# jchristopherson/nonlin

Hardware: AMD Instinct MI355X
Metric: LM iterations/sec on m=4096,n=256 fp64; FD-Jacobian GB/s vs HBM peak (higher is better)
Workload: dtype f64

## Files before the change

include/nonlin_hip.h:

```cpp
#ifndef NONLIN_HIP_H
#define NONLIN_HIP_H

#include <stdint.h>

#ifdef __cplusplus
extern "C" {
#endif

#define NLH_NO_ERROR                     0
#define NLH_INVALID_INPUT_ERROR        201
#define NLH_ARRAY_SIZE_ERROR           202
#define NLH_OUT_OF_MEMORY_ERROR        105
#define NLH_INVALID_OPERATION_ERROR    104
#define NLH_CONVERGENCE_ERROR          106
#define NLH_DIVERGENT_BEHAVIOR_ERROR   206
#define NLH_SPURIOUS_CONVERGENCE_ERROR 207
#define NLH_TOLERANCE_TOO_SMALL_ERROR  208
#define NLH_DIVIDE_BY_ZERO_ERROR       210
#define NLH_UNDEFINED_FUNCTION_ERROR   211
#define NLH_UNDERDEFINED_PROBLEM_ERROR 212
#define NLH_ERR_NO_DEVICE             -1
#define NLH_ERR_HIP                   -2
#define NLH_ERR_BAD_HANDLE            -3

// ... 205 lines not shown
                    double *dA, double *db, double *dxtrue, double *dx0);


int nlh_dq_residual(nlh_handle *h, int32_t nprob, int32_t m, int32_t n, const double *dA,
                    const double *db, double gamma, const double *dx, double *df);
int nlh_dq_fd_panel(nlh_handle *h, int32_t nprob, int32_t m, int32_t n, const double *dA,
                    const double *db, double gamma, const double *dx, double *dP);
int nlh_fd_jacobian_panel(nlh_handle *h, int32_t nprob, int32_t m, int32_t n,
                          const double *dP, const double *df0, const double *dx, double *dJ);
int nlh_dq_jacobian(nlh_handle *h, int32_t nprob, int32_t m, int32_t n, const double *dA,
                    double gamma, const double *dx, double *dJ);
int nlh_gram(nlh_handle *h, int32_t nprob, int32_t m, int32_t n, const double *dJ,
             const double *df, double *dG, double *dg);
int nlh_chol_factor(nlh_handle *h, int32_t nprob, int32_t n, double *dG, const double *dg,
                    int32_t *dipvt, double *dacnorm, double *dqtf, int32_t *dinfo);
int nlh_qr_factor(nlh_handle *h, int32_t nprob, int32_t m, int32_t n, double *dJ,
                  const double *df, int32_t *dipvt, double *drdiag, double *dacnorm,
                  double *dqtf, double *dwa4);
int nlh_lmfactor_exact(nlh_handle *h, int32_t nprob, int32_t m, int32_t n, const double *dJ,
                       const double *df, double *dR, int32_t *dipvt, double *drdiag, double *dacnorm,
                       double *dqtf, double *dwa4);
enum { NLH_QRX_SWEEP_COLUMN = 0,
       NLH_QRX_SWEEP_LANE = 1 };
enum { NLH_QRX_INIT_SPLIT = 0,
       NLH_QRX_INIT_FUSED = 1 };
enum { NLH_QRX_PIVOT_FEW32 = 0,
       NLH_QRX_PIVOT_BATCH32 = 1,
       NLH_QRX_PIVOT_FEW64 = 2,
       NLH_QRX_PIVOT_BATCH64 = 3,
       NLH_QRX_PIVOT_LONG = 4,
       NLH_QRX_PIVOT_LONG_SCALED = 5,
       NLH_QRX_PIVOT_LONG_SPLIT = 6 };
enum { NLH_QRX_PASS_COLUMN = 0,
       NLH_QRX_PASS_WIDE = 1,
       NLH_QRX_PASS_WIDE_HALF = 2,
       NLH_QRX_PASS_FOUR_WAVE = 3,
       NLH_QRX_PASS_WAVE = 4,
       NLH_QRX_PASS_WAVE_SHARED = 5 };
typedef struct nlh_qrx_plan_head {
    int32_t sweep, init;
    int32_t use_list, ny;
    int32_t nact;
} nlh_qrx_plan_head;
typedef struct nlh_qrx_plan_step {
    int32_t j, cur, np;
    int32_t lo;
    int32_t flush, pf;
    int32_t pivot, pass;
    int32_t gwin;
    int32_t lds, lds_max;
} nlh_qrx_plan_step;
int32_t nlh_qrx_plan(int32_t nprob, int32_t m, int32_t n, int32_t nact, int32_t have_stages,
                     nlh_qrx_plan_head *head, nlh_qrx_plan_step *steps, int32_t cap);
int nlh_lmpar(nlh_handle *h, int32_t nprob, int32_t n, double *dR, int32_t ldr,
              const int32_t *dipvt, const double *ddiag, const double *dqtf,
              const double *ddelta, const double *dtailsq, double *dpar,
              double *dxstep, double *dsdiag);
int nlh_lu_factor(nlh_handle *h, int32_t nprob, int32_t n, double *dA, int32_t *dipvt,
                  int32_t *dinfo);
int nlh_lu_solve(nlh_handle *h, int32_t nprob, int32_t n, const double *dLU,
                 const int32_t *dipvt, double *db);
int nlh_qr_factor_full(nlh_handle *h, int32_t nprob, int32_t n, const double *dB, double *dQ,
                       double *dRt);
int nlh_qr_rank1_update(nlh_handle *h, int32_t nprob, int32_t n, double *dQ, double *dRt,
                        const double *du, const double *dv);
int nlh_solve_upper(nlh_handle *h, int32_t nprob, int32_t n, const double *dRt, double *dx);
int nlh_chol_rank1(nlh_handle *h, int32_t n, int32_t downdate, double *dRt, double *du, int32_t *hinfo);

int nlh_poly_fit(nlh_handle *h, int32_t npts, int32_t order, int32_t thru_zero, const double *x,
                 const double *y, double *coef);
int nlh_poly_fit_batch(nlh_handle *h, int32_t nprob, int32_t npts, int32_t order, int32_t thru_zero,
                       const double *dx, const double *dy, double *dcoef);

int nlh_poly_roots(nlh_handle *h, int32_t order, const double *coef, double *z, int32_t *info);
int nlh_poly_roots_batch(nlh_handle *h, int32_t nprob, int32_t order, const double *dcoef, double *dz,
                         int32_t *dinfo);
int nlh_poly_eval_batch(nlh_handle *h, int32_t nprob, int32_t order, int32_t npts, const double *dcoef,
                        const double *dx, double *dy);
int nlh_poly_eval_complex_batch(nlh_handle *h, int32_t nprob, int32_t order, int32_t npts, const double *dcoef,
                                const double *dz, double *dy);

int nlh_covar(nlh_handle *h, int32_t nprob, int32_t n, const double *dR, const int32_t *dipvt, double tol,
              double *dcov, int32_t *drank);
int64_t nlh_covar_lds_bytes(int32_t n);
int nlh_lm_covariance_batch_device(nlh_handle *h, int32_t nprob, int32_t m, int32_t n, nlh_device_vecfcn fcn,
                                   nlh_device_jacfcn jacfcn, void *ctx, const double *dx, int32_t scaled, double tol,
                                   double *dcov, double *dsigma, int32_t *drank, double *dchi2);
int nlh_lm_covariance_batch_device_h(nlh_handle *h, int32_t nprob, int32_t m, int32_t n, nlh_device_vecfcn fcn,
                                     nlh_device_jacfcn jacfcn, void *ctx, const double *x, int32_t scaled, double tol,
                                     double *cov, double *sigma, int32_t *rank, double *chi2);
int nlh_lm_covariance(nlh_handle *h, int32_t m, int32_t n, nlh_vecfcn fcn, nlh_jacfcn jacfcn, void *ctx, double *x,
                      int32_t scaled, double tol, double *cov, double *sigma, int32_t *rank, double *chi2);
int nlh_dq_model_lm_covariance(nlh_handle *h, const nlh_dq_model *model, const double *x, int32_t scaled, double tol,
                               double *cov, double *sigma, int32_t *rank, double *chi2);

#define NLH_CURVE_GAUSS     0
#define NLH_CURVE_LORENTZ   1
#define NLH_CURVE_EXPDECAY  2
#define NLH_CURVE_MAX_BASE  8
#define NLH_CURVE_MAX_N  8192
typedef struct nlh_curve_ctx {
    int32_t kind, ncomp, nbase;
    int32_t shared_t;
    int32_t m;
    const double *dt;
    const double *dy;
// ... 144 lines not shown
```

nonlin_amd/_lib.py:

```python
import ctypes as C
import os

_HERE = os.path.dirname(os.path.abspath(__file__))
LIB_PATH = os.path.join(_HERE, "libnonlin_hip.so")

c_double_p = C.POINTER(C.c_double)
c_int32_p = C.POINTER(C.c_int32)

VECFCN = C.CFUNCTYPE(None, C.c_void_p, C.c_int32, c_double_p, C.c_int32, c_double_p)
JACFCN = C.CFUNCTYPE(None, C.c_void_p, C.c_int32, c_double_p, C.c_int32, c_double_p)
FCNNVAR = C.CFUNCTYPE(C.c_double, C.c_void_p, C.c_int32, c_double_p)
GRADFCN = C.CFUNCTYPE(None, C.c_void_p, C.c_int32, c_double_p, c_double_p)
DEVFCN = C.CFUNCTYPE(C.c_int, C.c_void_p, C.c_void_p, C.c_int32, C.c_void_p, C.c_int32, C.c_void_p, C.c_int32, C.c_void_p)


class IterationBehavior(C.Structure):
    _fields_ = [(k, C.c_int32) for k in (
        "iter_count", "fcn_count", "jacobian_count", "gradient_count",
        "converge_on_fcn", "converge_on_chng", "converge_on_zero_diff")]

    def as_dict(self):
        return {k: int(getattr(self, k)) for k, _ in self._fields_}


# ... 32 lines not shown
SYMBOLS = {
    "nlh_default_options": (None, [C.POINTER(Options)]),
    "nlh_format_status": (C.c_int, [C.c_int32, C.c_int32, C.c_int32, C.c_double, C.c_double, C.c_char_p, C.c_int32]),
    "nlh_create": (C.c_int, [C.POINTER(_H), C.c_int32, C.c_void_p]),
    "nlh_destroy": (None, [_H]),
    "nlh_device_count": (C.c_int, []),
    "nlh_last_error": (C.c_char_p, [_H]),
    "nlh_version": (C.c_char_p, []),
    "nlh_fd_jacobian": (C.c_int, [_H, C.c_int32, C.c_int32, VECFCN, JACFCN, C.c_void_p, c_double_p, c_double_p, c_double_p]),
    "nlh_lm_solve": (C.c_int, [_H, C.POINTER(Options), C.c_int32, C.c_int32, VECFCN, JACFCN, C.c_void_p,
                               c_double_p, c_double_p, C.POINTER(IterationBehavior)]),
    "nlh_newton_solve": (C.c_int, [_H, C.POINTER(Options), C.c_int32, VECFCN, JACFCN, C.c_void_p,
                                   c_double_p, c_double_p, C.POINTER(IterationBehavior)]),
    "nlh_quasi_newton_solve": (C.c_int, [_H, C.POINTER(Options), C.c_int32, C.c_int32, VECFCN, JACFCN, C.c_void_p,
                                         c_double_p, c_double_p, C.POINTER(IterationBehavior)]),
    "nlh_cls_solve": (C.c_int, [_H, C.POINTER(Options), C.c_double, C.c_double, c_double_p, c_double_p, C.c_int32, C.c_int32,
                                VECFCN, JACFCN, C.c_void_p, c_double_p, c_double_p, C.POINTER(IterationBehavior)]),
    "nlh_fd_gradient": (C.c_int, [C.c_int32, FCNNVAR, GRADFCN, C.c_void_p, c_double_p, c_double_p, c_double_p]),
    "nlh_bfgs_solve": (C.c_int, [_H, C.POINTER(Options), C.c_int32, FCNNVAR, GRADFCN, C.c_void_p, c_double_p, c_double_p,
                                 C.POINTER(IterationBehavior)]),
    "nlh_dq_lm_solve_batch": (C.c_int, [_H, C.POINTER(Options), C.c_int32, C.c_int32, C.c_int32, C.c_void_p,
                                        C.c_void_p, C.c_double, C.c_void_p, C.c_void_p,
                                        C.POINTER(IterationBehavior), c_int32_p]),
    "nlh_dq_newton_solve_batch": (C.c_int, [_H, C.POINTER(Options), C.c_int32, C.c_int32, C.c_void_p, C.c_void_p,
                                            C.c_double, C.c_int32, C.c_void_p, C.c_void_p,
                                            C.POINTER(IterationBehavior), c_int32_p]),
    "nlh_dq_quasi_newton_solve_batch": (C.c_int, [_H, C.POINTER(Options), C.c_int32, C.c_int32, C.c_int32, C.c_void_p,
                                                  C.c_void_p, C.c_double, C.c_int32, C.c_void_p, C.c_void_p,
                                                  C.POINTER(IterationBehavior), c_int32_p]),
    "nlh_dq_cls_solve_batch": (C.c_int, [_H, C.POINTER(Options), C.c_double, C.c_double, c_double_p, c_double_p, C.c_int32,
                                         C.c_int32, C.c_int32, C.c_void_p, C.c_void_p, C.c_double, C.c_void_p, C.c_void_p,
                                         C.POINTER(IterationBehavior), c_int32_p]),
    "nlh_dq_bfgs_solve_batch": (C.c_int, [_H, C.POINTER(Options), C.c_int32, C.c_int32, C.c_int32, C.c_void_p, C.c_void_p,
                                          C.c_double, C.c_void_p, c_double_p, C.POINTER(IterationBehavior), c_int32_p]),
    "nlh_dq_generate": (C.c_int, [_H, C.c_int32, C.c_int32, C.c_int32, C.c_uint64, C.c_uint64, C.c_double, C.c_double,
                                  C.c_double, C.c_int32, C.c_void_p, C.c_void_p, C.c_void_p, C.c_void_p]),
    "nlh_dq_residual": (C.c_int, [_H, C.c_int32, C.c_int32, C.c_int32, C.c_void_p, C.c_void_p, C.c_double,
                                  C.c_void_p, C.c_void_p]),
    "nlh_dq_fd_panel": (C.c_int, [_H, C.c_int32, C.c_int32, C.c_int32, C.c_void_p, C.c_void_p, C.c_double,
                                  C.c_void_p, C.c_void_p]),
    "nlh_fd_jacobian_panel": (C.c_int, [_H, C.c_int32, C.c_int32, C.c_int32, C.c_void_p, C.c_void_p,
                                        C.c_void_p, C.c_void_p]),
    "nlh_dq_jacobian": (C.c_int, [_H, C.c_int32, C.c_int32, C.c_int32, C.c_void_p, C.c_double, C.c_void_p,
                                  C.c_void_p]),
    "nlh_gram": (C.c_int, [_H, C.c_int32, C.c_int32, C.c_int32, C.c_void_p, C.c_void_p, C.c_void_p, C.c_void_p]),
    "nlh_chol_factor": (C.c_int, [_H, C.c_int32, C.c_int32, C.c_void_p, C.c_void_p, C.c_void_p, C.c_void_p,
                                  C.c_void_p, C.c_void_p]),
    "nlh_qr_factor": (C.c_int, [_H, C.c_int32, C.c_int32, C.c_int32, C.c_void_p, C.c_void_p, C.c_void_p,
                                C.c_void_p, C.c_void_p, C.c_void_p, C.c_void_p]),
    "nlh_lmfactor_exact": (C.c_int, [_H, C.c_int32, C.c_int32, C.c_int32, C.c_void_p, C.c_void_p, C.c_void_p,
                                     C.c_void_p, C.c_void_p, C.c_void_p, C.c_void_p, C.c_void_p]),
    "nlh_qrx_plan": (C.c_int32, [C.c_int32, C.c_int32, C.c_int32, C.c_int32, C.c_int32, C.POINTER(QrxPlanHead),
                                 C.POINTER(QrxPlanStep), C.c_int32]),
    "nlh_lmpar": (C.c_int, [_H, C.c_int32, C.c_int32, C.c_void_p, C.c_int32, C.c_void_p, C.c_void_p, C.c_void_p,
                            C.c_void_p, C.c_void_p, C.c_void_p, C.c_void_p, C.c_void_p]),
    "nlh_lu_factor": (C.c_int, [_H, C.c_int32, C.c_int32, C.c_void_p, C.c_void_p, C.c_void_p]),
    "nlh_lu_solve": (C.c_int, [_H, C.c_int32, C.c_int32, C.c_void_p, C.c_void_p, C.c_void_p]),
    "nlh_qr_factor_full": (C.c_int, [_H, C.c_int32, C.c_int32, C.c_void_p, C.c_void_p, C.c_void_p]),
    "nlh_qr_rank1_update": (C.c_int, [_H, C.c_int32, C.c_int32, C.c_void_p, C.c_void_p, C.c_void_p, C.c_void_p]),
    "nlh_solve_upper": (C.c_int, [_H, C.c_int32, C.c_int32, C.c_void_p, C.c_void_p]),
    "nlh_chol_rank1": (C.c_int, [_H, C.c_int32, C.c_int32, C.c_void_p, C.c_void_p, c_int32_p]),
    "nlh_poly_fit": (C.c_int, [_H, C.c_int32, C.c_int32, C.c_int32, c_double_p, c_double_p, c_double_p]),
    "nlh_poly_fit_batch": (C.c_int, [_H, C.c_int32, C.c_int32, C.c_int32, C.c_int32, C.c_void_p, C.c_void_p, C.c_void_p]),
    "nlh_poly_roots": (C.c_int, [_H, C.c_int32, c_double_p, c_double_p, C.POINTER(C.c_int32)]),
    "nlh_poly_roots_batch": (C.c_int, [_H, C.c_int32, C.c_int32, C.c_void_p, C.c_void_p, C.c_void_p]),
    "nlh_poly_eval_batch": (C.c_int, [_H, C.c_int32, C.c_int32, C.c_int32, C.c_void_p, C.c_void_p, C.c_void_p]),
    "nlh_poly_eval_complex_batch": (C.c_int, [_H, C.c_int32, C.c_int32, C.c_int32, C.c_void_p, C.c_void_p, C.c_void_p]),
    "nlh_dq_model_create": (C.c_int, [_H, C.c_int32, C.c_int32, C.c_int32, c_double_p, c_double_p, C.c_double, C.POINTER(C.c_void_p)]),
    "nlh_device_set_create": (C.c_int, [C.POINTER(C.c_void_p), c_int32_p, C.c_int32]),
    "nlh_device_set_destroy": (None, [C.c_void_p]),
    "nlh_device_set_size": (C.c_int32, [C.c_void_p]),
    "nlh_device_set_handle": (C.c_void_p, [C.c_void_p, C.c_int32]),
    "nlh_device_set_last_error": (C.c_char_p, [C.c_void_p]),
    "nlh_dq_model_create_on": (C.c_int, [C.c_void_p, C.c_int32, C.c_int32, C.c_int32, c_double_p, c_double_p, C.c_double,
                                         C.POINTER(C.c_void_p)]),
    "nlh_dq_model_device_count": (C.c_int32, [C.c_void_p]),
    "nlh_dq_model_destroy": (None, [C.c_void_p]),
    "nlh_dq_model_shape": (None, [C.c_void_p, c_int32_p, c_int32_p, c_int32_p]),
    "nlh_dq_model_eval": (C.c_int, [_H, C.c_void_p, c_double_p, c_double_p]),
    "nlh_dq_model_lm_solve": (C.c_int, [_H, C.POINTER(Options), C.c_void_p, c_double_p, c_double_p,
                                        C.POINTER(IterationBehavior), c_int32_p]),
    "nlh_dq_model_newton_solve": (C.c_int, [_H, C.POINTER(Options), C.c_void_p, C.c_int32, c_double_p, c_double_p,
                                            C.POINTER(IterationBehavior), c_int32_p]),
    "nlh_dq_model_quasi_newton_solve": (C.c_int, [_H, C.POINTER(Options), C.c_void_p, C.c_int32, C.c_int32, c_double_p, c_double_p,
                                                  C.POINTER(IterationBehavior), c_int32_p]),
    "nlh_dq_model_cls_solve": (C.c_int, [_H, C.POINTER(Options), C.c_void_p, C.c_double, C.c_double, c_double_p, c_double_p,
                                         c_double_p, c_double_p, C.POINTER(IterationBehavior), c_int32_p]),
    "nlh_dq_model_bfgs_solve": (C.c_int, [_H, C.POINTER(Options), C.c_void_p, c_double_p, c_double_p, c_double_p,
                                          C.POINTER(IterationBehavior), c_int32_p]),
    "nlh_fd_jacobian_device": (C.c_int, [_H, C.c_int32, C.c_int32, C.c_int32, DEVFCN, DEVFCN, C.c_void_p, C.c_void_p, C.c_void_p,
                                         C.c_void_p]),
    "nlh_lm_solve_batch_device": (C.c_int, [_H, C.POINTER(Options), C.c_int32, C.c_int32, C.c_int32, DEVFCN, DEVFCN, C.c_void_p,
                                            C.c_void_p, C.c_void_p, C.POINTER(IterationBehavior), c_int32_p]),
    "nlh_newton_solve_batch_device": (C.c_int, [_H, C.POINTER(Options), C.c_int32, C.c_int32, DEVFCN, DEVFCN, C.c_void_p,
                                                C.c_void_p, C.c_void_p, C.POINTER(IterationBehavior), c_int32_p]),
    "nlh_quasi_newton_solve_batch_device": (C.c_int, [_H, C.POINTER(Options), C.c_int32, C.c_int32, C.c_int32, DEVFCN, DEVFCN,
                                                      C.c_void_p, C.c_void_p, C.c_void_p, C.POINTER(IterationBehavior), c_int32_p]),
    "nlh_cls_solve_batch_device": (C.c_int, [_H, C.POINTER(Options), C.c_double, C.c_double, c_double_p, c_double_p, C.c_int32, C.c_int32,
                                             C.c_int32, DEVFCN, DEVFCN, C.c_void_p, C.c_void_p, C.c_void_p,
                                             C.POINTER(IterationBehavior), c_int32_p]),
    "nlh_cls_solve_batch_device_h": (C.c_int, [_H, C.POINTER(Options), C.c_double, C.c_double, c_double_p, c_double_p, C.c_int32, C.c_int32,
                                               C.c_int32, DEVFCN, DEVFCN, C.c_void_p, c_double_p, c_double_p,
                                               C.POINTER(IterationBehavior), c_int32_p]),
    "nlh_bfgs_solve_batch_device": (C.c_int, [_H, C.POINTER(Options), C.c_int32, C.c_int32, DEVFCN, DEVFCN, C.c_void_p, C.c_void_p, c_double_p,
                                              C.POINTER(IterationBehavior), c_int32_p]),
    "nlh_bfgs_solve_batch_device_h": (C.c_int, [_H, C.POINTER(Options), C.c_int32, C.c_int32, DEVFCN, DEVFCN, C.c_void_p, c_double_p, c_double_p,
# ... 330 lines not shown
```

nonlin_amd/csrc/nlh_common.h:

```cpp
#pragma once
#include <hip/hip_runtime.h>
#include <stdint.h>
#include <type_traits>

#define NLH_WAVE 64

enum NlhStage : int32_t {
    ST_NEED_JAC = 0,
    ST_HAVE_JAC = 1,
    ST_NE_READY = 2,
    ST_NEED_QR = 3,
    ST_QR_READY = 4,
    ST_TRIAL_READY = 5,
    ST_TRIAL_DONE = 6,
    ST_DONE = 7,
    ST_NEED_PCHOL = 8
};

struct LmState {
    double fnorm, fnorm1, par, delta, xnorm, gnorm, pnorm;
    double temp1n;
    double tailsq;
    int32_t iter, neval, njac;
    int32_t stage;
// ... 471 lines not shown
    __syncthreads();
    const double r = carry[0] * sqrt(1.0 + carry[1]);
    __syncthreads();
    return r;
}

__device__ __forceinline__ void nlh_lds_barrier() { asm volatile("s_waitcnt lgkmcnt(0)\n\ts_barrier" ::: "memory"); }

__device__ __forceinline__ bool nlh_odd_ulps(double c, double inv2ulp)
{
    const double z = c * inv2ulp;
    return z != floor(z);
}
template <int EL>
__device__ __forceinline__ double ordered_possum_wave_int(const double (&d)[EL], double s0, bool &ok)
{
    const long long sb = __double_as_longlong(s0);
    const long long es = sb >> 52;
    const double ulp = __longlong_as_double((es - 52) << 52), hu = 0.5 * ulp, inv2ulp = 0.5 / ulp;
    const double C = __longlong_as_double((es << 52) | (1ll << 51)), lim = 0.25 * __longlong_as_double(es << 52);
    double c0 = 0.0, c1 = 0.0;
    bool fine = true;
#pragma unroll
    for (int u = 0; u < EL; ++u) {
        const double x = d[u];
        fine = fine && (x <= lim);
        const double t = C + x, q = t - C, r = x - q;
        const bool tie = fabs(r) == hu;
        if (__builtin_expect(__builtin_amdgcn_ballot_w64(tie) != 0ull, 0)) {
            const double f = x - hu;
            const double a0 = tie ? f + (nlh_odd_ulps(c0 + f, inv2ulp) ? ulp : 0.0) : q;
            const double a1 = tie ? f + (nlh_odd_ulps(c1 + f, inv2ulp) ? 0.0 : ulp) : q;
            c0 = c0 + a0;
            c1 = c1 + a1;
        } else {
            c0 = c0 + q;
            c1 = c1 + q;
        }
    }
#pragma unroll
    for (int off = 1; off < 64; off <<= 1) {
        const double r0 = __shfl_down(c0, off, 64), r1 = __shfl_down(c1, off, 64);
        const double n0 = c0 + (nlh_odd_ulps(c0, inv2ulp) ? r1 : r0);
        const double n1 = c1 + (nlh_odd_ulps(c1, inv2ulp) ? r0 : r1);
        c0 = n0; c1 = n1;
    }
    const double totl = (sb & 1ll) ? c1 : c0;
    const double tot = __hiloint2double(__builtin_amdgcn_readfirstlane(__double2hiint(totl)), __builtin_amdgcn_readfirstlane(__double2loint(totl)));
    const double out = s0 + tot;
    ok = (__builtin_amdgcn_ballot_w64(!fine) == 0ull) && ((__double_as_longlong(out) >> 52) == es);
    return out;
}

template <int EL, int BSZ, typename Get>
__device__ double norm2_flang_block_lanes_pipe(Get get, int len, double *cd, double *aux, double *wm)
{
    constexpr int CAP = 64 * EL, PADCAP = CAP + 128, E = CAP / BSZ, TPR = EL / E, nw = BSZ / 64;
    static_assert(CAP % BSZ == 0 && EL % E == 0 && E % 2 == 0, "chunk must split evenly");
    const int tid = threadIdx.x, lane = tid & 63, wid = tid >> 6;
    const bool prep = wid < nw, chain = (wid == nw);
    const int nch = (len + CAP - 1) / CAP, i0 = tid * E;
    int *tflags = reinterpret_cast<int *>(aux + 8);
    auto loadabs = [&](int c, double (&a)[E]) __attribute__((always_inline)) {
        const int base = c * CAP, cl = min(CAP, len - base);
#pragma unroll
        for (int u = 0; u < E; ++u) a[u] = (i0 + u < cl) ? fabs(get(base + i0 + u)) : 0.0;
    };
    auto scanmax = [&](int c, const double (&a)[E]) __attribute__((always_inline)) {
        double lm = 0.0;
#pragma unroll
        for (int u = 0; u < E; ++u) lm = fmax(lm, a[u]);
        double sc = lm;
#pragma unroll
        for (int off = 1; off < 64; off <<= 1) {
            const double o = __shfl_up(sc, off, 64);
            if (lane >= off) sc = fmax(sc, o);
        }
        double ex = __shfl_up(sc, 1, 64);
        if (lane == 0) ex = 0.0;
        if (lane == 63) wm[c * nw + wid] = sc;
        return ex;
    };
    double a0[E], a1[E], ex0 = 0.0;
    __syncthreads();
    if (prep) {
        loadabs(0, a0);
        if (nch > 1) loadabs(1, a1);
        ex0 = scanmax(0, a0);
    }
    __syncthreads();
    double mxrun = 0.0, s = 0.0;
    for (int c = 0; c < nch; ++c) {
        const int cl = min(CAP, len - c * CAP);
        double *dsv = cd + (size_t)(c & 1) * PADCAP;
        int *tf = tflags + (c & 1) * BSZ;
        double mxc = mxrun;
#pragma unroll
        for (int w = 0; w < nw; ++w) mxc = fmax(mxc, wm[c * nw + w]);
        if (prep) {
            double prev = fmax(mxrun, ex0);
#pragma unroll
            for (int w = 0; w < nw; ++w)
                if (w < wid) prev = fmax(prev, wm[c * nw + w]);
            unsigned newmax = 0;
            double2 *ddst = reinterpret_cast<double2 *>(dsv + i0 + 2 * (i0 / EL));
#pragma unroll
// ... 271 lines not shown
```

nonlin_amd/csrc/nlh_lm.hip:

```cpp
#include "nlh_internal.h"
#include <chrono>
#include "nlh_kernels_gram.h"
#include "nlh_kernels_factor.h"
#include "nlh_kernels_lm.h"
#include "nlh_kernels_exact.h"
#include "nlh_qrx.h"


static __global__ void k_lmpar_standalone(int n, double *Rall, int ldr, const int32_t *ipvt_all, const double *diag_all,
                                   const double *qtf_all, const double *delta_all, const double *tailsq_all,
                                   double *par_all, double *x_all, double *sdiag_all, double *Wall, int ringcap);



void nlh_lm_init_device(int lds_max)
{
    hipFuncSetAttribute((const void *)k_gram_tri<16>, hipFuncAttributeMaxDynamicSharedMemorySize, lds_max);
    hipFuncSetAttribute((const void *)k_gram_tri<8>, hipFuncAttributeMaxDynamicSharedMemorySize, lds_max);
    hipFuncSetAttribute((const void *)k_gram_512, hipFuncAttributeMaxDynamicSharedMemorySize, lds_max);
    hipFuncSetAttribute((const void *)k_chol_factor, hipFuncAttributeMaxDynamicSharedMemorySize, lds_max);
    hipFuncSetAttribute((const void *)k_chol_nopiv<16>, hipFuncAttributeMaxDynamicSharedMemorySize, lds_max);
    hipFuncSetAttribute((const void *)k_chol_mc_step<16>, hipFuncAttributeMaxDynamicSharedMemorySize, lds_max);
    hipFuncSetAttribute((const void *)k_qr_factor, hipFuncAttributeMaxDynamicSharedMemorySize, lds_max);
    hipFuncSetAttribute((const void *)k_lmpar<false>, hipFuncAttributeMaxDynamicSharedMemorySize, lds_max);
// ... 667 lines not shown
    nlh_options o;
    nlh_default_options(&o);
    {
        Timed t(h, NLH_K_CHOL);
        size_t sh = sizeof(double) * (size_t)(3 * n + 64);
        hipLaunchKernelGGL(k_chol_factor, dim3(nprob), dim3(factor_threads(n)), sh, h->stream, n, dG,
                           (const double *)nullptr, dg, v, (const double *)nullptr, (LmState *)nullptr, dinfo,
                           o.factor, o.gtol, 0.0, 1, -1);
    }
    HIPCHK(h, hipGetLastError());
    return 0;
}

int nlh_qr_factor(nlh_handle *h, int32_t nprob, int32_t m, int32_t n, double *dJ, const double *df,
                  int32_t *dipvt, double *drdiag, double *dacnorm, double *dqtf, double *dwa4)
{
    if (!h) return NLH_ERR_BAD_HANDLE;
    HIPCHK(h, hipSetDevice(h->device));
    int rc;
    if ((rc = ensure(h, h->G, sizeof(double) * (size_t)nprob * n * n))) return rc;
    LmVecs v;
    memset(&v, 0, sizeof v);
    v.ipvt = dipvt; v.acnorm = dacnorm; v.qtf = dqtf; v.rdiag = drdiag;
    {
        Timed t(h, NLH_K_QR);
        size_t sh = sizeof(double) * (size_t)(3 * n + 64);
        hipLaunchKernelGGL(k_qr_factor, dim3(nprob), dim3(1024), sh, h->stream, m, n, dJ, df, (double *)h->G.p, v,
                           dwa4, dwa4, (const double *)nullptr, (LmState *)nullptr, 100.0, 0.0, 1);
    }
    HIPCHK(h, hipGetLastError());
    return 0;
}

int nlh_lmfactor_exact(nlh_handle *h, int32_t nprob, int32_t m, int32_t n, const double *dJ, const double *df,
                       double *dR, int32_t *dipvt, double *drdiag, double *dacnorm, double *dqtf, double *dwa4)
{
    if (!h) return NLH_ERR_BAD_HANDLE;
    if (nprob <= 0) return 0;
    if (m < n || n < 1) return NLH_INVALID_INPUT_ERROR;
    HIPCHK(h, hipSetDevice(h->device));
    int rc;
    if ((rc = ensure(h, h->P, sizeof(double) * qrx_matrix_doubles(nprob, m, n)))) return rc;
    if ((rc = ensure(h, h->qxV, qrx_workspace_bytes(nprob, m, n)))) return rc;
    LmVecs v;
    memset(&v, 0, sizeof v);
    v.ipvt = dipvt; v.acnorm = dacnorm; v.qtf = dqtf; v.rdiag = drdiag;
    if (qrx_factor(h->stream, nprob, m, n, dJ, (double *)h->P.p, df, dR, v, dwa4, dwa4, (const double *)nullptr, (LmState *)nullptr,
                   100.0, 0.0, h->qxV.p, (const QrxTimer *)nullptr, nprob))
        return qrx_no_launch(h);
    HIPCHK(h, hipGetLastError());
    return 0;
}


static __global__ void __launch_bounds__(1024)
k_lmpar_standalone(int n, double *Rall, int ldr, const int32_t *ipvt_all, const double *diag_all,
                   const double *qtf_all, const double *delta_all, const double *tailsq_all, double *par_all,
                   double *x_all, double *sdiag_all, double *Wall, int ringcap)
{
    extern __shared__ double smem[];
    const int p = blockIdx.x, tid = threadIdx.x, BS = blockDim.x;
    double *xs = smem, *sdiag = smem + n, *wa1 = smem + 2 * n, *wa2n = smem + 3 * n, *z = smem + 4 * n;
    double *red = smem + 5 * n;
    double *rot = red + 64;
    double par = par_all[p];
    lmpar_dev<false>(n, n, Rall + (size_t)p * ldr * n, ldr, ipvt_all + (size_t)p * n, diag_all + (size_t)p * n,
                     qtf_all + (size_t)p * n, delta_all[p], &par, tailsq_all[p], nullptr, xs, sdiag, wa1, wa2n, z,
                     red, nullptr, Wall + (size_t)p * n * n, rot, 0, ringcap > 0 ? smem + 6 * n + 72 : nullptr, ringcap);
    __syncthreads();
    for (int j = tid; j < n; j += BS) {
        x_all[(size_t)p * n + j] = xs[j];
        sdiag_all[(size_t)p * n + j] = sdiag[j];
    }
    if (tid == 0) par_all[p] = par;
}


int nlh_lmpar(nlh_handle *h, int32_t nprob, int32_t n, double *dR, int32_t ldr, const int32_t *dipvt,
              const double *ddiag, const double *dqtf, const double *ddelta, const double *dtailsq,
              double *dpar, double *dxstep, double *dsdiag)
{
    if (!h) return NLH_ERR_BAD_HANDLE;
    if (nprob <= 0) return 0;
    if (n < 1) return NLH_INVALID_INPUT_ERROR;
    int cap;
    const size_t rb = lm_ring_bytes(n, lmpar_threads(n), &cap);
    const size_t sh = sizeof(double) * (size_t)(6 * n + 72) + rb;
    if (!lds_fits((const void *)k_lmpar_standalone, sh)) return NLH_ARRAY_SIZE_ERROR;
    HIPCHK(h, hipSetDevice(h->device));
    int rc = ensure(h, h->misc, sizeof(double) * (size_t)nprob * n * n);
    if (rc) return rc;
    {
        Timed t(h, NLH_K_LMPAR);
        hipLaunchKernelGGL(k_lmpar_standalone, dim3(nprob), dim3(lmpar_threads(n)), sh, h->stream, n, dR, ldr, dipvt,
                           ddiag, dqtf, ddelta, dtailsq, dpar, dxstep, dsdiag, (double *)h->misc.p, cap);
    }
    HIPCHK(h, hipGetLastError());
    return 0;
}
```

nonlin_amd/csrc/nlh_qrx.hip:

```cpp
#include "nlh_qrx.h"
#include "nlh_common.h"
#include "../../include/nonlin_hip.h"
#include <type_traits>
#include <cstdio>
#include <cstdlib>
#include <algorithm>

#ifndef QRX_C
#define QRX_C 10
#endif
#define QRX_TR 64
#define QRX_PAD_ROWS 160
#ifndef QRX_AUX_LOAD
#define QRX_AUX_LOAD 0
#endif
#ifndef QRX_AUX_STORE
#define QRX_AUX_STORE 1
#endif
#ifndef QRX_UF
#define QRX_UF(flush) 16
#endif

typedef unsigned int qrx_u32x2 __attribute__((ext_vector_type(2)));
typedef unsigned int qrx_u32x4 __attribute__((ext_vector_type(4)));
// ... 343 lines not shown
            const int i0 = j + tid + it * 4 * BS;
            if (i0 < m) {
                double e[4];
                gather4(i0, e);
#pragma unroll
                for (int u = 0; u < 4; ++u) {
                    keep[it * 4 + u] = e[u];
                    if (i0 + u * BS < m) stage[spos(i0 + u * BS - j)] = e[u];
                }
            }
        }
    } else if (LONG && np <= 1 && !move0) {
        const int jb = j & ~7, npair = (m - jb + 1) >> 1;
        const double *colp = Tp + qrx_at(jb, srck, ld);
        const size_t blk = (size_t)ld * 8;
        const double t0 = np ? tk[0] : 0.0;
        constexpr int GU = QRX_LONG_GU;
        for (int pb = tid; pb < npair; pb += GU * BS) {
            double2 ax[GU], px[GU];
#pragma unroll
            for (int u = 0; u < GU; ++u) {
                const int pr = min(pb + u * BS, npair - 1);
                ax[u] = *reinterpret_cast<const double2 *>(colp + (size_t)(pr >> 2) * blk + 2 * (pr & 3));
                px[u] = np ? *reinterpret_cast<const double2 *>(Vc + jb + 2 * pr) : make_double2(0.0, 0.0);
            }
#pragma unroll
            for (int u = 0; u < GU; ++u) {
                const int pr = pb + u * BS, row = jb + 2 * pr;
                if (pr >= npair) continue;
                if (np) { ax[u].x = ax[u].x - t0 * px[u].x; ax[u].y = ax[u].y - t0 * px[u].y; }
                if (row >= j && row + 1 < m) *reinterpret_cast<double2 *>(Vn + row) = ax[u];
                else {
                    if (row >= j && row < m) Vn[row] = ax[u].x;
                    if (row + 1 >= j && row + 1 < m) Vn[row + 1] = ax[u].y;
                }
            }
        }
    } else {
        for (int i0 = j + tid; i0 < m; i0 += 4 * BS) {
            double e[4];
            gather4(i0, e);
#pragma unroll
            for (int u = 0; u < 4; ++u)
                if (i0 + u * BS < m) Vn[i0 + u * BS] = e[u];
        }
    }
    __syncthreads();
    const double ejj = staged ? stage[0] : Vn[j];
#ifdef QRX_DBG_CLK
    clk[2] = wall_clock64();
#endif
    double ajnorm;
    if constexpr (LONG) ajnorm = norm2_flang_block_lanes_pipe<QRX_LONG_EL, 192>([&](int i) { return Vn[j + i]; }, m - j, cd, aux, wmx);
    else ajnorm = staged ? norm2_flang_block_lanes<QRX_NL, 256, FEW>([&](int i) { return stage[spos(i)]; }, m - j, cd, aux)
                         : norm2_flang_block_lanes<QRX_NL, 256, FEW>([&](int i) { return Vn[j + i]; }, m - j, cd, aux);
#ifdef QRX_DBG_CLK
    clk[3] = wall_clock64();
#endif
    double ajj = 0.0;
    if (staged) {
        if (ajnorm != 0.0 && ejj < 0.0) ajnorm = -ajnorm;
        const double dn = (ajnorm != 0.0) ? ajnorm : 1.0;
#pragma unroll
        for (int u = 0; u < KEEP; ++u) keep[u] = keep[u] / dn;
#pragma unroll
        for (int u = 0; u < KEEP; ++u) {
            const int i = j + tid + u * BS;
            double t = keep[u];
            if (ajnorm != 0.0 && i == j) { t = t + 1.0; ajj = t; }
            if (i < m) Vn[i] = t;
        }
    } else if (LONG && (flush & 4) && ajnorm != 0.0) {
        if (ejj < 0.0) ajnorm = -ajnorm;
        if (tid == 0) { ajj = ejj / ajnorm + 1.0; Vn[j] = ajj; }
    } else if (LONG && ajnorm != 0.0) {
        if (ejj < 0.0) ajnorm = -ajnorm;
        const int jb = j & ~7, nsec = (m - jb + 7) >> 3;
        for (int sb = tid; sb < nsec; sb += QRX_LONG_SU * BS) {
            double2 tx[QRX_LONG_SU][4];
#pragma unroll
            for (int q = 0; q < QRX_LONG_SU; ++q) {
                const double2 *sp = reinterpret_cast<const double2 *>(Vn + jb + (size_t)min(sb + q * BS, nsec - 1) * 8);
#pragma unroll
                for (int h = 0; h < 4; ++h) tx[q][h] = sp[h];
            }
#pragma unroll
            for (int q = 0; q < QRX_LONG_SU; ++q) {
                const int sc = sb + q * BS, row = jb + sc * 8;
                if (sc >= nsec) continue;
#pragma unroll
                for (int h = 0; h < 4; ++h) {
                    tx[q][h].x = tx[q][h].x / ajnorm;
                    tx[q][h].y = tx[q][h].y / ajnorm;
                    if (row + 2 * h == j) { tx[q][h].x = tx[q][h].x + 1.0; ajj = tx[q][h].x; }
                    if (row + 2 * h + 1 == j) { tx[q][h].y = tx[q][h].y + 1.0; ajj = tx[q][h].y; }
                }
                if (row >= j && row + 8 <= m) {
                    double2 *dp = reinterpret_cast<double2 *>(Vn + row);
#pragma unroll
                    for (int h = 0; h < 4; ++h) dp[h] = tx[q][h];
                } else {
#pragma unroll
                    for (int h = 0; h < 4; ++h) {
                        if (row + 2 * h >= j && row + 2 * h < m) Vn[row + 2 * h] = tx[q][h].x;
                        if (row + 2 * h + 1 >= j && row + 2 * h + 1 < m) Vn[row + 2 * h + 1] = tx[q][h].y;
                    }
                }
            }
// ... 1375 lines not shown
```

nonlin_amd/device.py:

```python
import ctypes as C

import numpy as np
import torch

from . import _lib

IB_DTYPE = np.dtype([(k, np.int32) for k, _ in _lib.IterationBehavior._fields_])


from ._lib import CURVE_GAUSS, CURVE_LORENTZ, CURVE_EXPDECAY, CURVE_KINDS, curve_kind, curve_nparams
from ._lib import Expr
from ._lib import ParamMap


def _chk(t, shape, name):
    if not (t.is_cuda and t.dtype == torch.float64 and t.is_contiguous() and tuple(t.shape) == tuple(shape)):
        raise ValueError(f"{name}: expected contiguous float64 GPU tensor of shape {tuple(shape)}, "
                         f"got {t.dtype} {tuple(t.shape)} cuda={t.is_cuda}")


QRX_SWEEPS = ("column", "lane")
QRX_INITS = ("split", "fused")
QRX_PIVOT_FORMS = ("few32", "batch32", "few64", "batch64", "long", "long_scaled", "long_split")
QRX_PASS_FORMS = ("column", "wide", "wide_half", "four_wave", "wave", "wave_shared")
# ... 515 lines not shown
        nprob, n, m = A.shape
        J = torch.empty_like(A)
        self.h.check(self.lib.nlh_dq_jacobian(self.h.ptr, nprob, m, n, A.data_ptr(), float(gamma), x.data_ptr(),
                                              J.data_ptr()), "nlh_dq_jacobian")
        return J

    def gram(self, J, f):
        nprob, n, m = J.shape
        G = torch.empty((nprob, n, n), dtype=torch.float64, device=J.device)
        g = torch.empty((nprob, n), dtype=torch.float64, device=J.device)
        self.h.check(self.lib.nlh_gram(self.h.ptr, nprob, m, n, J.data_ptr(), f.data_ptr(), G.data_ptr(),
                                       g.data_ptr()), "nlh_gram")
        return G, g

    def chol_factor(self, G, g):
        nprob, n, _ = G.shape
        dev = G.device
        ipvt = torch.empty((nprob, n), dtype=torch.int32, device=dev)
        acnorm = torch.empty((nprob, n), dtype=torch.float64, device=dev)
        qtf = torch.empty((nprob, n), dtype=torch.float64, device=dev)
        info = torch.empty((nprob,), dtype=torch.int32, device=dev)
        self.h.check(self.lib.nlh_chol_factor(self.h.ptr, nprob, n, G.data_ptr(), g.data_ptr(), ipvt.data_ptr(),
                                              acnorm.data_ptr(), qtf.data_ptr(), info.data_ptr()), "nlh_chol_factor")
        return ipvt, acnorm, qtf, info

    def qr_factor(self, J, f):
        nprob, n, m = J.shape
        dev = J.device
        ipvt = torch.empty((nprob, n), dtype=torch.int32, device=dev)
        rdiag = torch.empty((nprob, n), dtype=torch.float64, device=dev)
        acnorm = torch.empty((nprob, n), dtype=torch.float64, device=dev)
        qtf = torch.empty((nprob, n), dtype=torch.float64, device=dev)
        wa4 = torch.empty((nprob, m), dtype=torch.float64, device=dev)
        self.h.check(self.lib.nlh_qr_factor(self.h.ptr, nprob, m, n, J.data_ptr(), f.data_ptr(), ipvt.data_ptr(),
                                            rdiag.data_ptr(), acnorm.data_ptr(), qtf.data_ptr(), wa4.data_ptr()),
                     "nlh_qr_factor")
        return ipvt, rdiag, acnorm, qtf, wa4

    def lmfactor_exact(self, J, f):
        nprob, n, m = J.shape
        _chk(J, (nprob, n, m), "J"); _chk(f, (nprob, m), "f")
        dev = J.device
        R = torch.zeros((nprob, n, n), dtype=torch.float64, device=dev)
        ipvt = torch.empty((nprob, n), dtype=torch.int32, device=dev)
        rdiag = torch.empty((nprob, n), dtype=torch.float64, device=dev)
        acnorm = torch.empty((nprob, n), dtype=torch.float64, device=dev)
        qtf = torch.empty((nprob, n), dtype=torch.float64, device=dev)
        wa4 = torch.empty((nprob, m), dtype=torch.float64, device=dev)
        self.h.check(self.lib.nlh_lmfactor_exact(self.h.ptr, nprob, m, n, J.data_ptr(), f.data_ptr(), R.data_ptr(),
                                                 ipvt.data_ptr(), rdiag.data_ptr(), acnorm.data_ptr(), qtf.data_ptr(),
                                                 wa4.data_ptr()), "nlh_lmfactor_exact")
        return R, ipvt, rdiag, acnorm, qtf, wa4

    def lmpar(self, R, ipvt, diag, qtf, delta, tailsq, par):
        nprob, n, ldr = R.shape
        dev = R.device
        for t, nm in ((R, "R"), (diag, "diag"), (qtf, "qtf"), (delta, "delta"), (tailsq, "tailsq"), (par, "par")):
            if t.dtype != torch.float64 or not t.is_cuda:
                raise ValueError(f"{nm} must be a float64 GPU tensor")
        x = torch.empty((nprob, n), dtype=torch.float64, device=dev)
        sdiag = torch.empty((nprob, n), dtype=torch.float64, device=dev)
        par = par.clone()
        self.h.check(self.lib.nlh_lmpar(self.h.ptr, nprob, n, R.data_ptr(), ldr, ipvt.data_ptr(), diag.data_ptr(),
                                        qtf.data_ptr(), delta.data_ptr(), tailsq.data_ptr(), par.data_ptr(),
                                        x.data_ptr(), sdiag.data_ptr()), "nlh_lmpar")
        return par, x, sdiag

    def lu_factor(self, A):
        nprob, n, _ = A.shape
        ipvt = torch.empty((nprob, n), dtype=torch.int32, device=A.device)
        info = torch.empty((nprob,), dtype=torch.int32, device=A.device)
        self.h.check(self.lib.nlh_lu_factor(self.h.ptr, nprob, n, A.data_ptr(), ipvt.data_ptr(), info.data_ptr()),
                     "nlh_lu_factor")
        return ipvt, info

    def qr_factor_full(self, B):
        nprob, n, _ = B.shape
        _chk(B, (nprob, n, n), "B")
        Q = torch.empty_like(B)
        Rt = torch.empty_like(B)
        self.h.check(self.lib.nlh_qr_factor_full(self.h.ptr, nprob, n, B.data_ptr(), Q.data_ptr(), Rt.data_ptr()),
                     "nlh_qr_factor_full")
        return Q, Rt

    def qr_rank1_update(self, Q, Rt, u, v):
        nprob, n, _ = Q.shape
        _chk(Q, (nprob, n, n), "Q"); _chk(Rt, (nprob, n, n), "Rt"); _chk(u, (nprob, n), "u"); _chk(v, (nprob, n), "v")
        self.h.check(self.lib.nlh_qr_rank1_update(self.h.ptr, nprob, n, Q.data_ptr(), Rt.data_ptr(), u.data_ptr(),
                                                  v.data_ptr()), "nlh_qr_rank1_update")
        return Q, Rt

    def solve_upper(self, Rt, x):
        nprob, n, _ = Rt.shape
        _chk(Rt, (nprob, n, n), "Rt"); _chk(x, (nprob, n), "x")
        self.h.check(self.lib.nlh_solve_upper(self.h.ptr, nprob, n, Rt.data_ptr(), x.data_ptr()), "nlh_solve_upper")
        return x

    def poly_fit_batch(self, x, y, order, thru_zero=False):
        nprob, npts = x.shape
        _chk(x, (nprob, npts), "x"); _chk(y, (nprob, npts), "y")
        coef = torch.empty((nprob, order + 1), dtype=torch.float64, device=x.device)
        rc = self.lib.nlh_poly_fit_batch(self.h.ptr, nprob, npts, int(order), int(thru_zero), x.data_ptr(), y.data_ptr(),
                                         coef.data_ptr())
        self.h.check(rc, "nlh_poly_fit_batch")
        if rc:
            raise RuntimeError(f"nlh_poly_fit_batch returned {rc}")
# ... 225 lines not shown
```

Before: 3770.

## Use segmented exact-rounding parallel norm2 in non-long QR column path

Replaces the lane-based serial scaled 2-norm in the non-LONG QR column step with a new block algorithm. It computes the running-max scaled terms in parallel and, when the partial sums stay within one binade, does exact round-to-nearest-even parallel accumulation with paired odd/even carries. It falls back to a serial handoff across waves only for segments that cannot be summed that way, with a retry if the exponent guard fails. This aims to shorten the serial dependency chain of the Fortran-order norm while keeping bitwise-identical results, at the cost of more barriers, shuffles and a possible second pass. A standalone kernel, Python binding and reference model are added for testing.

```diff
diff --git a/include/nonlin_hip.h b/include/nonlin_hip.h
--- a/include/nonlin_hip.h
+++ b/include/nonlin_hip.h
@@ -281,6 +281,8 @@
 } nlh_qrx_plan_step;
 int32_t nlh_qrx_plan(int32_t nprob, int32_t m, int32_t n, int32_t nact, int32_t have_stages,
                      nlh_qrx_plan_head *head, nlh_qrx_plan_step *steps, int32_t cap);
+int nlh_norm2_seg(nlh_handle *h, int32_t nvec, int32_t ld, int32_t el, const double *dx, const int32_t *dlens,
+                  double *dnorm, int32_t *dcnt);
 int nlh_lmpar(nlh_handle *h, int32_t nprob, int32_t n, double *dR, int32_t ldr,
               const int32_t *dipvt, const double *ddiag, const double *dqtf,
               const double *ddelta, const double *dtailsq, double *dpar,
diff --git a/nonlin_amd/_lib.py b/nonlin_amd/_lib.py
--- a/nonlin_amd/_lib.py
+++ b/nonlin_amd/_lib.py
@@ -108,6 +108,7 @@
                                      C.c_void_p, C.c_void_p, C.c_void_p, C.c_void_p, C.c_void_p]),
     "nlh_qrx_plan": (C.c_int32, [C.c_int32, C.c_int32, C.c_int32, C.c_int32, C.c_int32, C.POINTER(QrxPlanHead),
                                  C.POINTER(QrxPlanStep), C.c_int32]),
+    "nlh_norm2_seg": (C.c_int, [_H, C.c_int32, C.c_int32, C.c_int32, C.c_void_p, C.c_void_p, C.c_void_p, C.c_void_p]),
     "nlh_lmpar": (C.c_int, [_H, C.c_int32, C.c_int32, C.c_void_p, C.c_int32, C.c_void_p, C.c_void_p, C.c_void_p,
                             C.c_void_p, C.c_void_p, C.c_void_p, C.c_void_p, C.c_void_p]),
     "nlh_lu_factor": (C.c_int, [_H, C.c_int32, C.c_int32, C.c_void_p, C.c_void_p, C.c_void_p]),
diff --git a/nonlin_amd/csrc/nlh_common.h b/nonlin_amd/csrc/nlh_common.h
--- a/nonlin_amd/csrc/nlh_common.h
+++ b/nonlin_amd/csrc/nlh_common.h
@@ -547,6 +547,183 @@
     return out;
 }
 
+__device__ __forceinline__ double nlh_readlane_f64(double v, int l)
+{
+    return __hiloint2double(__builtin_amdgcn_readlane(__double2hiint(v), l), __builtin_amdgcn_readlane(__double2loint(v), l));
+}
+
+template <int EL, int BSZ, bool COUNT = false, typename Get>
+__device__ double norm2_flang_block_seg(Get get, int len, double *aux, int *cnt = nullptr)
+{
+    constexpr int CAP = 64 * EL, E = CAP / BSZ, nw = BSZ / 64;
+    static_assert(CAP % BSZ == 0 && E % 2 == 0 && E <= 32 && 4 * nw + 4 <= BSZ, "chunk must split evenly");
+    const int tid = threadIdx.x, lane = tid & 63, wid = tid >> 6;
+    double *wmax = aux, *carry = aux + 32, *hand = aux + 34, *wcd = aux + 40;
+    int *flag = reinterpret_cast<int *>(wcd + 2 * nw);
+    __syncthreads();
+    if (tid == 0) {
+        carry[0] = 0.0; carry[1] = 0.0;
+        if (COUNT) { flag[1] = 0; flag[2] = 0; flag[3] = 0; }
+    }
+    for (int base = 0; base < len; base += CAP) {
+        const int cl = min(CAP, len - base);
+        const int i0 = tid * E;
+        const bool act = i0 < cl;
+#pragma unroll 1
+        for (int attempt = 0; attempt < 2; ++attempt) {
+            double d[E], lm = 0.0;
+#pragma unroll
+            for (int u = 0; u < E; ++u) {
+                d[u] = (i0 + u < cl) ? fabs(get(base + i0 + u)) : 0.0;
+                lm = fmax(lm, d[u]);
+            }
+            double sc = lm;
+#pragma unroll
+            for (int off = 1; off < 64; off <<= 1) {
+                const double o = __shfl_up(sc, off, 64);
+                if (lane >= off) sc = fmax(sc, o);
+            }
+            double ex = __shfl_up(sc, 1, 64);
+            if (lane == 0) ex = 0.0;
+            __syncthreads();
+            if (lane == 63) wmax[wid] = sc;
+            if (tid == 0) flag[0] = 0;
+            __syncthreads();
+            const double mx_in = carry[0], s_in = carry[1];
+            double prev = fmax(mx_in, ex);
+            for (int w = 0; w < wid; ++w) prev = fmax(prev, wmax[w]);
+            unsigned nm = 0;
+#pragma unroll
+            for (int u = 0; u < E; ++u) {
+                const double av = d[u];
+                const bool gt = av > prev;
+                const double t = (gt ? prev : av) / (gt ? av : prev), tsq = t * t;
+                if (gt && prev != 0.0 && tsq != 1.0) nm |= 1u << u;
+                d[u] = (prev == 0.0) ? 0.0 : tsq;
+                prev = fmax(prev, av);
+            }
+            double mC = 1.0, mD = 0.0;
+#pragma unroll
+            for (int u = 0; u < E; ++u) {
+                const double c = ((nm >> u) & 1u) ? d[u] : 1.0;
+                mC = mC * c;
+                mD = mD * c + d[u];
+            }
+            double sC = mC, sD = mD;
+#pragma unroll
+            for (int off = 1; off < 64; off <<= 1) {
+                const double oC = __shfl_up(sC, off, 64), oD = __shfl_up(sD, off, 64);
+                if (lane >= off) { sD = oD * sC + sD; sC = oC * sC; }
+            }
+            double xC = __shfl_up(sC, 1, 64), xD = __shfl_up(sD, 1, 64);
+            if (lane == 0) { xC = 1.0; xD = 0.0; }
+            if (lane == 63) { wcd[wid] = sC; wcd[nw + wid] = sD; }
+            __syncthreads();
+            double sh = s_in;
+            for (int w = 0; w < wid; ++w) sh = sh * wcd[w] + wcd[nw + w];
+            const double shin = sh * xC + xD, shout = shin * mC + mD;
+            constexpr double G = 9.313225746154785e-10;
+            const long long ea = __double_as_longlong(shin * (1.0 - G)) >> 52, eb = __double_as_longlong(shin * (1.0 + G)) >> 52,
+                            ec = __double_as_longlong(shout * (1.0 + G)) >> 52;
+            const bool fre = attempt == 0 && act && nm == 0 && shin >= 4.0 && ea == eb && eb == ec;
+            const long long es = fre ? ea : 1025ll;
+            const double ulp = __longlong_as_double((es - 52) << 52), hu = 0.5 * ulp, inv2ulp = 0.5 / ulp;
+            const double C = __longlong_as_double((es << 52) | (1ll << 51));
+            double c0 = 0.0, c1 = 0.0;
+#pragma unroll
+            for (int u = 0; u < E; ++u) {
+                const double x = d[u];
+                const double t = C + x, q = t - C, r = x - q;
+                const bool tie = fabs(r) == hu;
+                if (__builtin_expect(__builtin_amdgcn_ballot_w64(tie) != 0ull, 0)) {
+                    const double f = x - hu;
+                    const double a0 = tie ? f + (nlh_odd_ulps(c0 + f, inv2ulp) ? ulp : 0.0) : q;
+                    const double a1 = tie ? f + (nlh_odd_ulps(c1 + f, inv2ulp) ? 0.0 : ulp) : q;
+                    c0 = c0 + a0;
+                    c1 = c1 + a1;
+                } else {
+                    c0 = c0 + q;
+                    c1 = c1 + q;
+                }
+            }
+            if (fre) {
+#pragma unroll
+                for (int u = 0; u < E; ++u) d[u] = 0.0;
+            } else {
+                c0 = 0.0; c1 = 0.0;
+            }
+            const int el = fre ? (int)es : -1;
+            const int pel = __shfl_up(el, 1, 64);
+            const bool head = act && (lane == 0 || !fre || pel != el);
+            const unsigned long long heads = __builtin_amdgcn_ballot_w64(head);
+            const int rid = fre ? 63 - __clzll((long long)(heads & ((2ull << lane) - 1ull))) : -1 - lane;
+#pragma unroll
+            for (int off = 1; off < 64; off <<= 1) {
+                const double r0 = __shfl_down(c0, off, 64), r1 = __shfl_down(c1, off, 64);
+                const int prid = __shfl_down(rid, off, 64);
+                if (lane + off < 64 && prid == rid) {
+                    const double n0 = c0 + (nlh_odd_ulps(c0, inv2ulp) ? r1 : r0);
+                    const double n1 = c1 + (nlh_odd_ulps(c1, inv2ulp) ? r0 : r1);
+                    c0 = n0; c1 = n1;
+                }
+            }
+#pragma unroll 1
+            for (int w = 0; w < nw; ++w) {
+                if (wid == w && flag[0] == 0) {
+                    double s = nlh_readlane_f64(w ? hand[0] : s_in, 0);
+                    int nterm = 0, nitem = 0;
+                    int badl = 0;
+                    unsigned long long todo = heads;
+#pragma unroll 1
+                    while (todo != 0ull) {
+                        const int L = __builtin_amdgcn_readfirstlane(__ffsll((long long)todo) - 1);
+                        todo &= todo - 1ull;
+                        const unsigned nml = (unsigned)__builtin_amdgcn_readlane((int)nm, L);
+                        double t = s + ((__double2loint(s) & 1) ? c1 : c0);
+                        badl |= (int)(lane == L) & (int)(el >= 0) & ((int)((__double2hiint(s) >> 20) != el) | (int)((__double2hiint(t) >> 20) != el));
+                        if (__builtin_expect(nml == 0u, 1)) {
+#pragma unroll
+                            for (int u = 0; u < E; ++u) t = t + d[u];
+                        } else {
+#pragma unroll
+                            for (int u = 0; u < E; ++u) {
+                                t = t * (((nml >> u) & 1u) ? d[u] : 1.0);
+                                t = t + d[u];
+                            }
+                        }
+                        s = nlh_readlane_f64(t, L);
+                        if (COUNT) {
+                            ++nitem;
+                            if (__builtin_amdgcn_readlane(el, L) < 0) nterm += min(E, cl - (w * 64 + L) * E);
+                        }
+                    }
+                    const bool bad = __builtin_amdgcn_ballot_w64(badl != 0) != 0ull;
+                    if (lane == 0) {
+                        hand[0] = s;
+                        if (bad) flag[0] = 1;
+                        if (COUNT) { flag[1] += nterm; flag[2] += nitem; if (bad) flag[3] = 1; }
+                    }
+                }
+                __syncthreads();
+            }
+            if (flag[0] == 0) {
+                if (tid == 0) {
+                    double mx = mx_in;
+                    for (int w = 0; w < nw; ++w) mx = fmax(mx, wmax[w]);
+                    carry[0] = mx;
+                    carry[1] = hand[0];
+                }
+                break;
+            }
+        }
+    }
+    __syncthreads();
+    const double r = carry[0] * sqrt(1.0 + carry[1]);
+    if (COUNT && tid == 0) { cnt[0] = flag[1]; cnt[1] = flag[2]; cnt[2] = flag[3]; }
+    __syncthreads();
+    return r;
+}
+
 template <int EL, int BSZ, typename Get>
 __device__ double norm2_flang_block_lanes_pipe(Get get, int len, double *cd, double *aux, double *wm)
 {
diff --git a/nonlin_amd/csrc/nlh_lm.hip b/nonlin_amd/csrc/nlh_lm.hip
--- a/nonlin_amd/csrc/nlh_lm.hip
+++ b/nonlin_amd/csrc/nlh_lm.hip
@@ -743,6 +743,30 @@
     return 0;
 }
 
+template <int EL>
+static __global__ void __launch_bounds__(256)
+k_norm2_seg(int ld, const double *__restrict__ x, const int32_t *__restrict__ lens, double *__restrict__ nrm, int32_t *__restrict__ cnt)
+{
+    __shared__ __attribute__((aligned(16))) double aux[40 + 128];
+    const int v = blockIdx.x;
+    const double *xv = x + (size_t)v * ld;
+    const double r = norm2_flang_block_seg<EL, 256, true>([&](int i) { return xv[i]; }, min(max(lens[v], 0), ld), aux, cnt + 3 * (size_t)v);
+    if (threadIdx.x == 0) nrm[v] = r;
+}
+
+int nlh_norm2_seg(nlh_handle *h, int32_t nvec, int32_t ld, int32_t el, const double *dx, const int32_t *dlens, double *dnorm,
+                  int32_t *dcnt)
+{
+    if (!h) return NLH_ERR_BAD_HANDLE;
+    if (nvec <= 0) return 0;
+    if (ld < 1 || (el != 32 && el != 64)) return NLH_INVALID_INPUT_ERROR;
+    HIPCHK(h, hipSetDevice(h->device));
+    if (el == 32) hipLaunchKernelGGL(k_norm2_seg<32>, dim3(nvec), dim3(256), 0, h->stream, ld, dx, dlens, dnorm, dcnt);
+    else hipLaunchKernelGGL(k_norm2_seg<64>, dim3(nvec), dim3(256), 0, h->stream, ld, dx, dlens, dnorm, dcnt);
+    HIPCHK(h, hipGetLastError());
+    return 0;
+}
+
 
 static __global__ void __launch_bounds__(1024)
 k_lmpar_standalone(int n, double *Rall, int ldr, const int32_t *ipvt_all, const double *diag_all,
diff --git a/nonlin_amd/csrc/nlh_qrx.hip b/nonlin_amd/csrc/nlh_qrx.hip
--- a/nonlin_amd/csrc/nlh_qrx.hip
+++ b/nonlin_amd/csrc/nlh_qrx.hip
@@ -419,8 +419,8 @@
 #endif
     double ajnorm;
     if constexpr (LONG) ajnorm = norm2_flang_block_lanes_pipe<QRX_LONG_EL, 192>([&](int i) { return Vn[j + i]; }, m - j, cd, aux, wmx);
-    else ajnorm = staged ? norm2_flang_block_lanes<QRX_NL, 256, FEW>([&](int i) { return stage[spos(i)]; }, m - j, cd, aux)
-                         : norm2_flang_block_lanes<QRX_NL, 256, FEW>([&](int i) { return Vn[j + i]; }, m - j, cd, aux);
+    else ajnorm = staged ? norm2_flang_block_seg<QRX_NL, 256>([&](int i) { return stage[spos(i)]; }, m - j, aux)
+                         : norm2_flang_block_seg<QRX_NL, 256>([&](int i) { return Vn[j + i]; }, m - j, aux);
 #ifdef QRX_DBG_CLK
     clk[3] = wall_clock64();
 #endif
diff --git a/nonlin_amd/device.py b/nonlin_amd/device.py
--- a/nonlin_amd/device.py
+++ b/nonlin_amd/device.py
@@ -591,6 +591,17 @@
                                                  wa4.data_ptr()), "nlh_lmfactor_exact")
         return R, ipvt, rdiag, acnorm, qtf, wa4
 
+    def norm2_seg(self, x, lens, el=64):
+        nvec, ld = x.shape
+        _chk(x, (nvec, ld), "x")
+        if lens.dtype != torch.int32 or not lens.is_cuda or tuple(lens.shape) != (nvec,) or not lens.is_contiguous():
+            raise ValueError("lens must be a contiguous int32 GPU tensor of shape (nvec,)")
+        nrm = torch.empty((nvec,), dtype=torch.float64, device=x.device)
+        cnt = torch.zeros((nvec, 3), dtype=torch.int32, device=x.device)
+        self.h.check(self.lib.nlh_norm2_seg(self.h.ptr, nvec, ld, int(el), x.data_ptr(), lens.data_ptr(), nrm.data_ptr(),
+                                            cnt.data_ptr()), "nlh_norm2_seg")
+        return nrm, cnt
+
     def lmpar(self, R, ipvt, diag, qtf, delta, tailsq, par):
         nprob, n, ldr = R.shape
         dev = R.device
diff --git a/profiles/ubench/norm2_seg.py b/profiles/ubench/norm2_seg.py
--- /dev/null
+++ b/profiles/ubench/norm2_seg.py
@@ -0,0 +1,140 @@
+import math
+import struct
+
+import numpy as np
+
+GUARD = 2.0 ** -30
+
+
+def _bits(x):
+    return struct.unpack("<q", struct.pack("<d", x))[0]
+
+
+def _expo(x):
+    return _bits(x) >> 52
+
+
+def _odd(c, inv2ulp):
+    z = c * inv2ulp
+    return z != math.floor(z)
+
+
+def terms(x, mx=0.0):
+    a = np.abs(np.asarray(x, dtype=np.float64))
+    d = np.zeros(a.size)
+    f = np.zeros(a.size, dtype=bool)
+    prev = float(mx)
+    for i, av in enumerate(a.tolist()):
+        gt = av > prev
+        if prev != 0.0:
+            num, den = (prev, av) if gt else (av, prev)
+            t = num / den
+            tsq = t * t
+            d[i] = tsq
+            f[i] = gt and tsq != 1.0
+        prev = max(prev, av)
+    return d, f, prev
+
+
+def chain(d, f, s=0.0):
+    for di, fi in zip(d.tolist(), f.tolist()):
+        if fi:
+            s = s * di
+        s = s + di
+    return s
+
+
+def thread_pair(d, es):
+    ulp = 2.0 ** (es - 1023 - 52)
+    hu, inv2ulp = 0.5 * ulp, 0.5 / ulp
+    C = 1.5 * 2.0 ** (es - 1023)
+    c0 = c1 = 0.0
+    for x in d.tolist():
+        t = C + x
+        q = t - C
+        r = x - q
+        if abs(r) == hu:
+            fl = x - hu
+            a0 = fl + (ulp if _odd(c0 + fl, inv2ulp) else 0.0)
+            a1 = fl + (0.0 if _odd(c1 + fl, inv2ulp) else ulp)
+            c0, c1 = c0 + a0, c1 + a1
+        else:
+            c0, c1 = c0 + q, c1 + q
+    return c0, c1
+
+
+def fold(left, right, es):
+    inv2ulp = 0.5 / 2.0 ** (es - 1023 - 52)
+    return (left[0] + (right[1] if _odd(left[0], inv2ulp) else right[0]),
+            left[1] + (right[0] if _odd(left[1], inv2ulp) else right[1]))
+
+
+def chunk_sum(d, f, s_in, E, perturb=0.0, rng=None):
+    n = d.size
+    nthr = (n + E - 1) // E
+    sh = [s_in]
+    s = s_in
+    for g in range(nthr):
+        s = chain(d[g * E:(g + 1) * E], f[g * E:(g + 1) * E], s)
+        if perturb:
+            s *= 1.0 + rng.uniform(-1.0, 1.0) * perturb
+        sh.append(s)
+    items = []
+    for g in range(nthr):
+        lo, hi = g * E, min(n, (g + 1) * E)
+        shin, shout = sh[g], sh[g + 1]
+        ea, eb, ec = _expo(shin * (1.0 - GUARD)), _expo(shin * (1.0 + GUARD)), _expo(shout * (1.0 + GUARD))
+        free = (not f[lo:hi].any()) and shin >= 4.0 and ea == eb == ec
+        if not free:
+            items.append(("S", lo, hi))
+        elif g % 64 and items[-1][0] == "F" and items[-1][1] == ea:
+            items[-1] = ("F", ea, fold(items[-1][2], thread_pair(d[lo:hi], ea), ea))
+        else:
+            items.append(("F", ea, thread_pair(d[lo:hi], ea)))
+    s, nser, nit, ok = s_in, 0, 0, True
+    for it in items:
+        nit += 1
+        if it[0] == "S":
+            s = chain(d[it[1]:it[2]], f[it[1]:it[2]], s)
+            nser += it[2] - it[1]
+        else:
+            es, (c0, c1) = it[1], it[2]
+            s2 = s + (c1 if _bits(s) & 1 else c0)
+            if _expo(s) != es or _expo(s2) != es:
+                ok = False
+                break
+            s = s2
+    if not ok:
+        s = chain(d, f, s_in)
+        nser += n
+        nit += nthr
+    return s, nser, nit, not ok
+
+
+def norm2_seg(x, el=64, bsz=256, perturb=0.0, rng=None):
+    x = np.asarray(x, dtype=np.float64)
+    cap, E = 64 * el, 64 * el // bsz
+    mx, s, nser, nit, redone = 0.0, 0.0, 0, 0, False
+    for base in range(0, x.size, cap):
+        d, f, mx = terms(x[base:base + cap], mx)
+        s, a, b, c = chunk_sum(d, f, s, E, perturb, rng)
+        nser, nit, redone = nser + a, nit + b, redone or c
+    return mx * math.sqrt(1.0 + s), nser, nit, redone
+
+
+def norm2_plain(x):
+    d, f, mx = terms(x)
+    return mx * math.sqrt(1.0 + chain(d, f))
+
+
+if __name__ == "__main__":
+    rng = np.random.default_rng(1)
+    bad = tot = 0
+    for rep in range(10):
+        for n in (4096, 4095, 2049, 1031, 257, 17):
+            for a in (rng.standard_normal(n), rng.standard_cauchy(n), rng.integers(-8, 9, n) / 8.0,
+                      rng.choice([1.0, 0.5, 0.25, 2.0 ** -26, 2.0 ** -27], n)):
+                r, nser, nit, redone = norm2_seg(a, perturb=1e-13, rng=rng)
+                tot += 1
+                bad += r != norm2_plain(a)
+    print("vectors", tot, "mismatches", bad)
```

Result: no change. 3806 (median of 6 runs) (+1.0%).
